# bit-bots/SoccerDiffusion

Measured on AMD Instinct MI355X. Metric: denoised joint-trajectories/s (50-step DDIM, H=100, J=20), higher is better.
Workload: dtype f32 (operands split into fp16 hi+lo, 3 fp16 MFMAs per product at every site, fp32 accumulate: 22-bit operands; single noise prediction vs the fp64 oracle 8e-7 on these weights and 2e-6 on weights stressed to |logit| ~ 60 (tests/test_gpu_denoiser.py::test_mode3_noise_prediction_single_step); valid fo; 1 GPU; BASELINE.json configs[2]: 50-step DDIM sampling, B=4096 parallel rollouts per GPU, transformer denoiser d=256 L=4 heads=4, horizon T=100, J=20, memory M=11 (10 context tokens + step token); one step = one full rollout; the timed region issues the rollout's launches eagerly.  Kernel selection: sampler mode 3 (--sampler-mode); batch_per_gpu=4096, ddim_steps=50, horizon=100, joints=20, hidden_dim=256, decoder_layers=4, parallelism=dp1 (independent rollouts, no collective)

## Files before the change

soccerdiffusion_amd/csrc/sd_traj.h:

```cpp
#pragma once
#include "sd_common.h"
#include "sd_mfma16.h"
#include "soccerdiffusion_hip.h"
#include <type_traits>

namespace tj {

constexpr int D = 256, HD = 64, NH = 4, TMAX = 100;
constexpr int NTHREADS = 512;
constexpr int MAX_L = 8;
constexpr float ACT = 8.0f;
constexpr float PSC = 1024.0f;
constexpr float XSC = 1.0f;
constexpr int XROW = 1024, X1ROW = 512, QROW = 256, VROW = 288, PROW = 512;
constexpr int LDS_X = 0;
constexpr int LDS_SQ = LDS_X + TMAX * X1ROW;
constexpr int LDS_SO = LDS_SQ + TMAX * QROW;
constexpr int LDS_Q = LDS_X + TMAX * XROW;
constexpr int LDS_K = LDS_Q + TMAX * QROW;
constexpr int LDS_P = LDS_Q;
constexpr int LDS_STAT = LDS_K + TMAX * VROW;
constexpr int LDS_BYTES = LDS_STAT + TMAX * 8 * 8;
static_assert(LDS_SO + TMAX * QROW <= LDS_Q, "Q and O fit the freed half of the panel");
static_assert(LDS_BYTES <= 163840 && LDS_P + TMAX * PROW <= LDS_STAT, "LDS budget");

typedef short s16x4 __attribute__((ext_vector_type(4)));
typedef _Float16 f16x2 __attribute__((ext_vector_type(2)));
typedef unsigned u32x4 __attribute__((ext_vector_type(4)));

#ifdef TJ_STAMPS
constexpr int TJ_NSTAMP = 96, TJ_STAMP_WGS = 512;
__device__ unsigned long long *g_tj_stamps;
#define TJ_STAMP(i)                                                                                                            \
    do {                                                                                                                       \
        if (blockIdx.x < TJ_STAMP_WGS && (threadIdx.x & 63) == 0)                                                              \
            g_tj_stamps[((long)blockIdx.x * 8 + (threadIdx.x >> 6)) * TJ_NSTAMP + (i)] = __builtin_amdgcn_s_memtime();        \
    } while (0)
template <int SITE>
__device__ __forceinline__ void tj_sync() {
    const unsigned long long t0 = __builtin_amdgcn_s_memtime();
    __syncthreads();
    const unsigned long long t1 = __builtin_amdgcn_s_memtime();
    if (blockIdx.x < TJ_STAMP_WGS && (threadIdx.x & 63) == 0) g_tj_stamps[((long)blockIdx.x * 8 + (threadIdx.x >> 6)) * TJ_NSTAMP + 64 + SITE] += t1 - t0;
}
#define TJ_SYNC(site) tj_sync<site>()
#define TJ_WAIT_FIRST_KEY() asm volatile("s_waitcnt vmcnt(28)" ::: "memory")
#else
#define TJ_STAMP(i) do {} while (0)
#define TJ_SYNC(site) __syncthreads()
#define TJ_WAIT_FIRST_KEY() do {} while (0)
#endif

#ifndef TJ_DROP_ALO
#define TJ_DROP_ALO 0
#endif
#ifndef TJ_DROP_BLO
#define TJ_DROP_BLO 0
#endif
enum Site { S_QKV = 1, S_SCORES = 2, S_PV = 4, S_OUT = 8, S_XSC = 16, S_XPV = 32, S_W1 = 64, S_W2 = 128, S_EMB = 256, S_FC = 512 };
template <int SITE = 0>
__device__ __forceinline__ void mma3(f32x4 &c, f16x8 ah, f16x8 al, f16x8 bh, f16x8 bl) {
    if constexpr ((TJ_DROP_ALO | TJ_DROP_BLO) & SITE) {
        if constexpr (!(TJ_DROP_ALO & SITE)) c = mfma16(al, bh, c);
        if constexpr (!(TJ_DROP_BLO & SITE)) c = mfma16(ah, bl, c);
        c = mfma16(ah, bh, c);
    } else {
        ::mma3(c, ah, al, bh, bl);
    }
}

__device__ __forceinline__ int kperm(int k8, int e) { return (k8 >> 2) * 32 + 16 * (e >> 2) + 4 * (k8 & 3) + (e & 3); }

static __global__ void pack_w16_kernel(const float *__restrict__ W, int N, int K, int Np, int Kp, const unsigned *maxbits, float fixed_scale,
                                f16 *__restrict__ dst, float *scale_out) {
    const float scale = maxbits ? f16_scale_from_bits(*maxbits) : fixed_scale;
    if (scale_out && blockIdx.x == 0 && threadIdx.x == 0) *scale_out = scale;
    const int nks = Kp / 32;
    const long total = (long)Np * (Kp / 8);
    for (long i = (long)blockIdx.x * blockDim.x + threadIdx.x; i < total; i += (long)gridDim.x * blockDim.x) {
        const int n = (int)(i / (Kp / 8)), k8 = (int)(i % (Kp / 8));
        f16 hh[8], ll[8];
#pragma unroll
        for (int e = 0; e < 8; ++e) {
            const int k = Kp == D ? kperm(k8, e) : k8 * 8 + e;
            const float v = (n < N && k < K) ? W[(long)n * K + k] * scale : 0.f;
            hh[e] = (f16)v;
            ll[e] = (f16)(v - (float)hh[e]);
        }
        const int nt = n >> 4, ks = k8 >> 2, lane = (k8 & 3) * 16 + (n & 15);
        f16 *o = dst + (((long)nt * nks + ks) * 2) * 512 + lane * 8;
#pragma unroll
        for (int e = 0; e < 8; ++e) {
            o[e] = hh[e];
            o[512 + e] = ll[e];
        }
    }
}

static __global__ void pack_g16_kernel(const float *__restrict__ gv, long items, int n_slots, const unsigned *maxbits, f16 *__restrict__ dst,
                                float *scale_out, int nkt = 1) {
    const float scale = f16_scale_from_bits(*maxbits);
    if (scale_out && blockIdx.x == 0 && threadIdx.x == 0) *scale_out = scale;
    const long total = items * 4 * 16 * (D / 8);
    for (long i = (long)blockIdx.x * blockDim.x + threadIdx.x; i < total; i += (long)gridDim.x * blockDim.x) {
        const int k8 = (int)(i % (D / 8)), slot = (int)((i / (D / 8)) % 16);
        const long ih = i / (D / 8) / 16;
        f16x4 h0 = {0, 0, 0, 0}, l0 = h0, h1 = h0, l1 = h0;
        if (16 * (int)((ih >> 2) % nkt) + slot < n_slots) {
            const float *row = gv + (ih * 16 + slot) * 2 * D + kperm(k8, 0);
            f16_split4(*reinterpret_cast<const f32x4 *>(row), scale, h0, l0);
            f16_split4(*reinterpret_cast<const f32x4 *>(row + 16), scale, h1, l1);
        }
        f16 *o = dst + ih * (8 * 2 * 512) + ((k8 >> 2) * 2) * 512 + ((k8 & 3) * 16 + slot) * 8;
        *reinterpret_cast<f16x4 *>(o) = h0;
        *reinterpret_cast<f16x4 *>(o + 4) = h1;
        *reinterpret_cast<f16x4 *>(o + 512) = l0;
        *reinterpret_cast<f16x4 *>(o + 516) = l1;
    }
}
static __global__ void pack_v16_kernel(const float *__restrict__ gv, long items, int n_slots, const unsigned *maxbits, f16 *__restrict__ dst,
                                float *scale_out, int nkt = 1) {
    const float scale = f16_scale_from_bits(*maxbits);
    if (scale_out && blockIdx.x == 0 && threadIdx.x == 0) *scale_out = scale;
    const long total = items * 16 * 2 * 64;
    for (long i = (long)blockIdx.x * blockDim.x + threadIdx.x; i < total; i += (long)gridDim.x * blockDim.x) {
        const int lane = (int)(i & 63), kk = (int)((i >> 6) & 1), nt = (int)((i >> 7) & 15);
        const long item = i >> 11;
        const int n = 16 * nt + (lane & 15), g = lane >> 4;
        f16 hh[8], ll[8];
#pragma unroll
        for (int e = 0; e < 8; ++e) {
            const int k = 32 * kk + 8 * g + e, head = k >> 4, slot = k & 15;
            const float v = 16 * (int)(item % nkt) + slot < n_slots ? gv[((item * 4 + head) * 16 + slot) * 2 * D + D + n] * scale : 0.f;
            hh[e] = (f16)v;
            ll[e] = (f16)(v - (float)hh[e]);
        }
        f16 *o = dst + (((item * 16 + nt) * 2 + kk) * 2) * 512 + lane * 8;
#pragma unroll
        for (int e = 0; e < 8; ++e) {
            o[e] = hh[e];
            o[512 + e] = ll[e];
        }
    }
}

struct Ctx {
    char *smem;
    int lane, w, g, t, T;
    int tok6;
    bool ok6;
    unsigned xa[4], xa6[4];
};

struct LnAffine { f32x4 w[2], b[2]; };
__device__ __forceinline__ void ln_affine_load(const Ctx &c, const float *ln_w, const float *ln_b, LnAffine &p) {
    __builtin_amdgcn_sched_barrier(0);
#pragma unroll
    for (int a = 0; a < 2; ++a) {
        p.w[a] = *reinterpret_cast<const f32x4 *>(ln_w + 32 * c.w + 16 * a + 4 * c.g);
        p.b[a] = *reinterpret_cast<const f32x4 *>(ln_b + 32 * c.w + 16 * a + 4 * c.g);
    }
    __builtin_amdgcn_sched_barrier(0);
}


template <int NSTEP, int DEPTH, class Load, class Mma>
__device__ __forceinline__ void ring_pipe(Load load, Mma mma) {
#pragma unroll
    for (int s = 0; s < DEPTH - 1; ++s)
        if (s < NSTEP) load(s);
#pragma unroll
    for (int s = 0; s < NSTEP; ++s) {
        if (s + DEPTH - 1 < NSTEP) load(s + DEPTH - 1);
        __builtin_amdgcn_sched_barrier(0);
        mma(s);
        __builtin_amdgcn_sched_barrier(0);
    }
// ... 198 lines not shown
        const f32x4 d0 = H[0][tt] - mw[tt], d1 = H[1][tt] - mw[tt];
        const f32x4 q4 = d0 * d0 + d1 * d1;
        qw[tt] = rows4_sum((q4[0] + q4[1]) + (q4[2] + q4[3]));
    }
    if (c.g == 0) {
#pragma unroll
        for (int tt = 0; tt < NTT; ++tt)
            if (tok_ok(c, tt)) *reinterpret_cast<f32x2 *>(stat + (tok_of(c, tt) * 8 + c.w) * 2) = f32x2{mw[tt], qw[tt]};
    }
    TJ_STAMP(49);
    TJ_SYNC(0);
    TJ_STAMP(50);
    char *scr = c.smem + LDS_P + c.w * 1280 + c.t * 80;
#pragma unroll
    for (int j = 0; j < (NTT > 4 ? 2 : 1); ++j) {
        const int tl = c.g + 4 * j;
        const float *sp = stat + (tl < NTT - 1 ? 16 * tl + c.t : c.tok6) * 16;
        const f32x4 p0 = *reinterpret_cast<const f32x4 *>(sp), p1 = *reinterpret_cast<const f32x4 *>(sp + 4);
        const f32x4 p2 = *reinterpret_cast<const f32x4 *>(sp + 8), p3 = *reinterpret_cast<const f32x4 *>(sp + 12);
        const float m = (((p0[0] + p0[2]) + (p1[0] + p1[2])) + ((p2[0] + p2[2]) + (p3[0] + p3[2]))) * 0.125f;
        const f32x4 e0 = f32x4{p0[0], p0[2], p1[0], p1[2]} - m, e1 = f32x4{p2[0], p2[2], p3[0], p3[2]} - m;
        const f32x4 ee = e0 * e0 + e1 * e1;
        const float m2 = (((p0[1] + p0[3]) + (p1[1] + p1[3])) + ((p2[1] + p2[3]) + (p3[1] + p3[3]))) + 32.0f * ((ee[0] + ee[1]) + (ee[2] + ee[3]));
        *reinterpret_cast<f32x2 *>(scr + 8 * tl) = f32x2{m, __builtin_amdgcn_rsqf(m2 * (1.0f / D) + SD_LN_EPS)};
    }
    __builtin_amdgcn_wave_barrier();
    float mean[NTT], rstd[NTT];
#pragma unroll
    for (int i = 0; i < (NTT + 1) / 2; ++i) {
        const f32x4 v = *reinterpret_cast<const f32x4 *>(scr + 16 * i);
        mean[2 * i] = v[0];
        rstd[2 * i] = v[1];
        if (2 * i + 1 < NTT) {
            mean[2 * i + 1] = v[2];
            rstd[2 * i + 1] = v[3];
        }
    }
    TJ_STAMP(51);
    const f32x4 gw0 = gwv[0] * ACT, gb0 = gbv[0] * ACT, gw1 = gwv[1] * ACT, gb1 = gbv[1] * ACT;
#pragma unroll
    for (int tt = 0; tt < NTT; ++tt) {
        const f32x4 y0 = ((H[0][tt] - mean[tt]) * rstd[tt]) * gw0 + gb0, y1 = ((H[1][tt] - mean[tt]) * rstd[tt]) * gw1 + gb1;
        if constexpr (HI_ONLY) store_x1(c, tt, y0, y1);
        else store_x(c, tt, y0, y1);
        if (rows_out && tok_ok(c, tt)) {
            const f32x4 u0 = y0 * (1.0f / ACT), u1 = y1 * (1.0f / ACT);
            float *at = rows_out + (long)tok_of(c, tt) * D + 32 * c.w + 4 * c.g;
            SD_NT_STORE(u0, reinterpret_cast<f32x4 *>(at));
            SD_NT_STORE(u1, reinterpret_cast<f32x4 *>(at + 16));
            if (amax) {
                const f32x4 m4 = f32x4{fmaxf(fabsf(u0[0]), fabsf(u1[0])), fmaxf(fabsf(u0[1]), fabsf(u1[1])), fmaxf(fabsf(u0[2]), fabsf(u1[2])), fmaxf(fabsf(u0[3]), fabsf(u1[3]))};
                *amax = fmaxf(*amax, fmaxf(fmaxf(m4[0], m4[1]), fmaxf(m4[2], m4[3])));
            }
        }
        __builtin_amdgcn_sched_barrier(0);
    }
    TJ_STAMP(52);
    TJ_SYNC(1);
}
template <bool HI_ONLY = false>
static __device__ __forceinline__ void layer_norm_to_x(const Ctx &c0, const f32x4 (&H)[2][NTT], const float *ln_w, const float *ln_b, float *rows_out = nullptr,
                                                       float *amax = nullptr) {
    LnAffine aff;
    ln_affine_load(c0, ln_w, ln_b, aff);
    layer_norm_to_x<HI_ONLY>(c0, H, aff, rows_out, amax);
}

template <int T0 = 0, int NT = NTT, class Body>
static __device__ __forceinline__ void gemm_pipe(const Ctx &c, const f16 *pa0, const f16 *pa1, Body body) {
    const char *X = c.smem + LDS_X;
    const unsigned lo = (unsigned)c.lane * 8;
    f16x8 a0[2][2], a1[2][2], b[2][2];
#pragma unroll
    for (int pl = 0; pl < 2; ++pl) {
        a0[0][pl] = *reinterpret_cast<const f16x8 *>(pa0 + lo + pl * 512);
        a1[0][pl] = *reinterpret_cast<const f16x8 *>(pa1 + lo + pl * 512);
        b[0][pl] = lds16(X + x_at(c, T0, pl, 0));
    }
#pragma unroll
    for (int ks = 0; ks < 8; ++ks) {
#pragma unroll
        for (int tt = T0; tt < T0 + NT; ++tt) {
            const int cur = (ks * NT + tt - T0) & 1, nxt = cur ^ 1;
            if (tt == T0 && ks + 1 < 8) {
#pragma unroll
                for (int pl = 0; pl < 2; ++pl) {
                    a0[(ks + 1) & 1][pl] = *reinterpret_cast<const f16x8 *>(pa0 + lo + ((ks + 1) * 2 + pl) * 512);
                    a1[(ks + 1) & 1][pl] = *reinterpret_cast<const f16x8 *>(pa1 + lo + ((ks + 1) * 2 + pl) * 512);
                }
            }
            const int nks = tt + 1 < T0 + NT ? ks : ks + 1, ntt = tt + 1 < T0 + NT ? tt + 1 : T0;
            if (nks < 8) {
#pragma unroll
                for (int pl = 0; pl < 2; ++pl) b[nxt][pl] = lds16(X + x_at(c, ntt, pl, nks));
            }
            __builtin_amdgcn_sched_barrier(0);
            body(tt, a0[ks & 1][0], a0[ks & 1][1], a1[ks & 1][0], a1[ks & 1][1], b[cur][0], b[cur][1]);
            __builtin_amdgcn_sched_barrier(0);
        }
    }
}

struct HeadAcc { f32x4 a0[NTT], a1[NH0]; };
template <bool odd>
static __device__ __forceinline__ void gemm_head(const Ctx &c, HeadAcc &acc, const f16 *pa0, const f16 *pa1) {
    const char *X = c.smem + LDS_X;
    const unsigned lo = (unsigned)c.lane * 8;
    f16x8 a0[2][2], a1[2][2], b[2];
#pragma unroll
    for (int pl = 0; pl < 2; ++pl) {
        a0[0][pl] = *reinterpret_cast<const f16x8 *>(pa0 + lo + pl * 512);
        a1[0][pl] = *reinterpret_cast<const f16x8 *>(pa1 + lo + pl * 512);
    }
    b[0] = lds16(X + x1_at(c, 0, 0));
#pragma unroll
    for (int ks = 0; ks < 8; ++ks) {
#pragma unroll
        for (int tt = 0; tt < NTT; ++tt) {
            const int cur = (ks * NTT + tt) & 1, nxt = cur ^ 1;
            if (tt == 0 && ks + 1 < 8) {
#pragma unroll
                for (int pl = 0; pl < 2; ++pl) {
                    a0[(ks + 1) & 1][pl] = *reinterpret_cast<const f16x8 *>(pa0 + lo + ((ks + 1) * 2 + pl) * 512);
                    a1[(ks + 1) & 1][pl] = *reinterpret_cast<const f16x8 *>(pa1 + lo + ((ks + 1) * 2 + pl) * 512);
                }
            }
            const int nks = tt + 1 < NTT ? ks : ks + 1, ntt = tt + 1 < NTT ? tt + 1 : 0;
            if (nks < 8) b[nxt] = lds16(X + x1_at(c, ntt, nks));
            __builtin_amdgcn_sched_barrier(0);
            acc.a0[tt] = mfma16(a0[ks & 1][1], b[cur], acc.a0[tt]);
            acc.a0[tt] = mfma16(a0[ks & 1][0], b[cur], acc.a0[tt]);
            if constexpr (!odd) {
                if (tt < NH0) {
                    acc.a1[tt] = mfma16(a1[ks & 1][1], b[cur], acc.a1[tt]);
                    acc.a1[tt] = mfma16(a1[ks & 1][0], b[cur], acc.a1[tt]);
                }
            } else if (tt >= NH0) {
                acc.a1[tt - NH0] = mfma16(a1[ks & 1][1], b[cur], acc.a1[tt - NH0]);
                acc.a1[tt - NH0] = mfma16(a1[ks & 1][0], b[cur], acc.a1[tt - NH0]);
            }
            __builtin_amdgcn_sched_barrier(0);
        }
    }
}

template <int SITE>
static __device__ __forceinline__ void gemm_x2(const Ctx &c, f32x4 (&acc)[2][NTT], const f16 *wmat) {
    const f16 *pa = wmat + (long)(2 * c.w) * (8 * 2 * 512);
    gemm_pipe(c, pa, pa + 8 * 2 * 512, [&](int tt, f16x8 a0h, f16x8 a0l, f16x8 a1h, f16x8 a1l, f16x8 bh, f16x8 bl) __attribute__((always_inline)) {
        mma3<SITE>(acc[0][tt], a0h, a0l, bh, bl);
        mma3<SITE>(acc[1][tt], a1h, a1l, bh, bl);
    });
}

static __device__ __forceinline__ void gemm_k64(const Ctx &c, f32x4 (&acc)[2][NTT], const AK64 &f, const char *Bbuf) {
    const f16x8 (&a)[2][2][2] = f.a;
    f16x8 b[3][2];
    ring_pipe<2 * NTT, 3>(
        [&](int s) __attribute__((always_inline)) {
            b[s % 3][0] = lds16(Bbuf + q_at(c, s >> 1, 0, s & 1));
            b[s % 3][1] = lds16(Bbuf + q_at(c, s >> 1, 1, s & 1));
        },
        [&](int s) __attribute__((always_inline)) {
            const int tt = s >> 1, kk = s & 1;
            mma3<S_OUT>(acc[0][tt], a[0][kk][0], a[0][kk][1], b[s % 3][0], b[s % 3][1]);
            mma3<S_OUT>(acc[1][tt], a[1][kk][0], a[1][kk][1], b[s % 3][0], b[s % 3][1]);
        });
}


static __device__ __forceinline__ void head_zero(HeadAcc &acc) {
#pragma unroll
    for (int tt = 0; tt < NTT; ++tt) acc.a0[tt] = f32x4{0.f, 0.f, 0.f, 0.f};
#pragma unroll
    for (int i = 0; i < NH0; ++i) acc.a1[i] = f32x4{0.f, 0.f, 0.f, 0.f};
}
static __device__ __forceinline__ void head_gemm(const Ctx &c0, const SaW &a, int h, HeadAcc &acc) {
    const Ctx c = ctx_local(c0);
    const int w = c.w;
    const int nt0 = (w < 4 ? 0 : 16) + 4 * h + (w & 3);
    const int nt1 = 32 + 4 * h + (w >> 1);
    head_zero(acc);
    if (w & 1) gemm_head<true>(c, acc, a.w_in + (long)nt0 * (8 * 2 * 512), a.w_in + (long)nt1 * (8 * 2 * 512));
    else gemm_head<false>(c, acc, a.w_in + (long)nt0 * (8 * 2 * 512), a.w_in + (long)nt1 * (8 * 2 * 512));
}
static __device__ __forceinline__ void head_write_qkv(const Ctx &c0, const SaW &a, int h, const HeadAcc &acc) {
    const Ctx c = ctx_local(c0);
    const int w = c.w, g = c.g, t = c.t, w3 = w & 3;
    const float c_in = 1.0f / a.s_in;
    {
        const f32x4 bv = *reinterpret_cast<const f32x4 *>(a.b_in + (w < 4 ? 0 : D) + HD * h + 16 * w3 + 4 * g) * ACT;
        char *dst = c.smem + (w < 4 ? LDS_SQ : LDS_Q);
        const int chunk = (2 * (w3 & 1) + (g >> 1)) | ((w3 >> 1) << 3);
#pragma unroll
        for (int tt = 0; tt < NTT; ++tt) {
            if (!tok_ok(c, tt)) continue;
            const int tok = tok_of(c, tt);
            split_store(dst + q_off(tok, chunk) + 8 * (g & 1), dst + q_off(tok, chunk | 4) + 8 * (g & 1), acc.a0[tt] * c_in + bv);
            __builtin_amdgcn_sched_barrier(0);
        }
    }
    {
        const f32x4 bv = *reinterpret_cast<const f32x4 *>(a.b_in + 2 * D + HD * h + 16 * (w >> 1) + 4 * g) * ACT;
        const int tt1 = (w & 1) ? NH0 : 0, n1 = (w & 1) ? NTT - NH0 : NH0;
#pragma unroll
        for (int i = 0; i < NH0; ++i) {
            if (i >= n1) continue;
            const int tok = 16 * (tt1 + i) + t;
            if (tok >= c.T) continue;
            char *at = c.smem + LDS_K + tok * VROW + 2 * (16 * (w >> 1) + 4 * g);
            split_store(at, at + 128, acc.a1[i] * c_in + bv);
        }
    }
}
static __device__ __forceinline__ void att_scores(const Ctx &c, const SaW &a, const char *Qb, const char *Kb, f32x4 (&S)[NTT], float &psum,
                                                  float *lse2 = nullptr) {
    const int w = c.w, g = c.g, t = c.t;
    {
        f16x8 qf[2][2];
        const int qtok = min(16 * w + t, c.T - 1);
#pragma unroll
        for (int kk = 0; kk < 2; ++kk)
#pragma unroll
            for (int pl = 0; pl < 2; ++pl) qf[kk][pl] = lds16(Qb + q_off(qtok, g | (pl << 2) | (kk << 3)));
#pragma unroll
        for (int kt = 0; kt < NTT; ++kt) S[kt] = f32x4{0.f, 0.f, 0.f, 0.f};
        f16x8 kf[4][2];
        ring_pipe<2 * NTT, 4>(
            [&](int s) __attribute__((always_inline)) {
                kf[s & 3][0] = lds16(Kb + q_at(c, s >> 1, 0, s & 1));
                kf[s & 3][1] = lds16(Kb + q_at(c, s >> 1, 1, s & 1));
            },
            [&](int s) __attribute__((always_inline)) { mma3<S_SCORES>(S[s >> 1], kf[s & 3][0], kf[s & 3][1], qf[s & 1][0], qf[s & 1][1]); });
    }
    const float c_s = a.scale_log2e / (ACT * ACT);
#pragma unroll
    for (int r = 0; r < 4; ++r)
        if (LAST0 + 4 * g + r >= c.T) S[NTT - 1][r] = -INFINITY;
    f32x4 m4 = S[0];
#pragma unroll
    for (int kt = 1; kt < NTT; ++kt) m4 = f32x4{fmaxf(m4[0], S[kt][0]), fmaxf(m4[1], S[kt][1]), fmaxf(m4[2], S[kt][2]), fmaxf(m4[3], S[kt][3])};
    const float m = rows4_max(fmaxf(fmaxf(m4[0], m4[1]), fmaxf(m4[2], m4[3])));
    if constexpr (!PRECISE) {
        if (a.status && __builtin_amdgcn_ballot_w64(fabsf(m) * c_s > SD_SHARP_LOGIT_LIMIT * 1.44269504088896340736f) != 0) {
            if (c.lane == 0) atomicOr(a.status, SD_STATUS_SHARP_LOGITS);
        }
    }
    const float mb = m * c_s - 10.0f;
    f32x4 ps = {0.f, 0.f, 0.f, 0.f};
#pragma unroll
    for (int kt = 0; kt < NTT; ++kt) {
        const f32x4 e = S[kt] * c_s - mb;
        S[kt] = f32x4{__builtin_amdgcn_exp2f(e[0]), __builtin_amdgcn_exp2f(e[1]), __builtin_amdgcn_exp2f(e[2]), __builtin_amdgcn_exp2f(e[3])};
        ps = ps + S[kt];
    }
    psum = rows4_sum((ps[0] + ps[1]) + (ps[2] + ps[3]));
    if (lse2) *lse2 = mb + __builtin_amdgcn_logf(psum);
}
template <bool SPLIT_UNDER = false>
static __device__ __forceinline__ void att_pv(const Ctx &c, const f32x4 (&S)[NTT], float psum, const char *Vb, char *Ob, float *rows_out = nullptr,
                                              int ld = 0, float *amax = nullptr) {
    const int w = c.w, g = c.g, t = c.t;
    f32x4 O[4];
#pragma unroll
    for (int ft = 0; ft < 4; ++ft) O[ft] = f32x4{0.f, 0.f, 0.f, 0.f};
    const int q4 = t >> 2, p4 = t & 3;
    const auto vload = [&](int s, f16x8 (&vf)[4][2]) __attribute__((always_inline)) {
        const int kp = s >> 2, ft = s & 3;
        const int r0 = min(32 * kp + 4 * g + q4, c.T - 1), r1 = min(32 * kp + 16 + 4 * g + q4, c.T - 1);
        const char *v0 = Vb + r0 * VROW + 8 * p4, *v1 = Vb + r1 * VROW + 8 * p4;
#pragma unroll
        for (int pn = 0; pn < 2; ++pn) {
            const s16x4 x0 = __builtin_amdgcn_ds_read_tr16_b64_v4i16((__attribute__((address_space(3))) s16x4 *)(v0 + pn * 128 + ft * 32));
            const s16x4 x1 = __builtin_amdgcn_ds_read_tr16_b64_v4i16((__attribute__((address_space(3))) s16x4 *)(v1 + pn * 128 + ft * 32));
            vf[s & 3][pn] = __builtin_shufflevector(__builtin_bit_cast(f16x4, x0), __builtin_bit_cast(f16x4, x1), 0, 1, 2, 3, 4, 5, 6, 7);
        }
    };
    if constexpr (SPLIT_UNDER) {
        f16x8 vf[4][2];
        unsigned ph[2][4], pl[2][4];
        const auto psplit = [&](int kp, int q) __attribute__((always_inline)) {
            const int kt = 2 * kp + (q >> 1);
            f16x2 h = {0, 0}, l = {0, 0};
            if (kt < NTT) {
                const f32x2 x = {S[kt < NTT ? kt : 0][2 * (q & 1)], S[kt < NTT ? kt : 0][2 * (q & 1) + 1]};
                h = __builtin_convertvector(x, f16x2);
                l = __builtin_convertvector(x - __builtin_convertvector(h, f32x2), f16x2);
            }
            ph[kp & 1][q] = __builtin_bit_cast(unsigned, h);
            pl[kp & 1][q] = __builtin_bit_cast(unsigned, l);
            if (kt < NTT) asm volatile("" : "+v"(ph[kp & 1][q]), "+v"(pl[kp & 1][q]));
        };
        const auto pfrag = [](const unsigned (&p)[4]) __attribute__((always_inline)) { return __builtin_bit_cast(f16x8, u32x4{p[0], p[1], p[2], p[3]}); };
#pragma unroll
        for (int q = 0; q < 4; ++q) psplit(0, q);
#pragma unroll
        for (int s = 0; s < 3; ++s) vload(s, vf);
#pragma unroll
        for (int s = 0; s < 4 * NKP; ++s) {
            const int kp = s >> 2;
            if (s + 3 < 4 * NKP) vload(s + 3, vf);
            __builtin_amdgcn_sched_barrier(0);
            mma3<S_PV>(O[s & 3], vf[s & 3][0], vf[s & 3][1], pfrag(ph[kp & 1]), pfrag(pl[kp & 1]));
            if (kp + 1 < NKP) {
                psplit(kp + 1, s & 3);
#pragma unroll
// ... 288 lines not shown
#pragma unroll
        for (int i = 0; i < NH0; ++i) {
            if (i >= n1) continue;
            const f32x4 p = S[kt][i];
            const int tt = tt1 + i, tok = tt < NTT - 1 ? 16 * tt + c.t : c.tok6;
            if (tt == NTT - 1 && !c.ok6) continue;
            const int chunk = (2 * (hh & 1) + (c.g >> 1)) | ((hh >> 1) << 3);
            split_store(Pb + p_off(tok, chunk) + 8 * (c.g & 1), Pb + p_off(tok, chunk | 4) + 8 * (c.g & 1), p * ss.m_c);
            if (kt == klast && c.g == (mcs >> 2)) {
                const float pv = p[mcs & 3] * ss.m_s;
                const f16 ph = (f16)pv, pl = (f16)(pv - (float)ph);
                const f16x8 z8h = {ph, 0, 0, 0, 0, 0, 0, 0}, z8l = {pl, 0, 0, 0, 0, 0, 0, 0};
                *reinterpret_cast<f16x8 *>(Pb + p_off(tok, hh | (2 << 3))) = z8h;
                *reinterpret_cast<f16x8 *>(Pb + p_off(tok, hh | 4 | (2 << 3))) = z8l;
            }
        }
        f16x8 av[2][3][2];
#pragma unroll
        for (int n = 0; n < 2; ++n) {
            const f16 *vp = L.v16 + (((traj * nkt + kt) * 16 + 2 * c.w + n) * 2) * (2 * 512) + c.lane * 8;
#pragma unroll
            for (int kk = 0; kk < 2; ++kk)
#pragma unroll
                for (int pl = 0; pl < 2; ++pl) av[n][kk][pl] = *reinterpret_cast<const f16x8 *>(vp + (kk * 2 + pl) * 512);
#pragma unroll
            for (int pl = 0; pl < 2; ++pl) {
                const f16 sv = vstep[(pl * 4 + c.g) * D + 16 * (2 * c.w + n) + c.t];
                av[n][2][pl] = f16x8{sv, 0, 0, 0, 0, 0, 0, 0};
            }
        }
        TJ_SYNC(5);
        f16x8 pb[3][2];
        if (kt == klast) {
            ring_pipe<3 * NTT, 3>(
                [&](int s) __attribute__((always_inline)) {
                    pb[s % 3][0] = lds16(Pb + p_at(c, s / 3, 0, s % 3));
                    pb[s % 3][1] = lds16(Pb + p_at(c, s / 3, 1, s % 3));
                },
                [&](int s) __attribute__((always_inline)) {
                    const int tt = s / 3, kk = s % 3;
                    mma3<S_XPV>(H[0][tt], av[0][kk][0], av[0][kk][1], pb[s % 3][0], pb[s % 3][1]);
                    mma3<S_XPV>(H[1][tt], av[1][kk][0], av[1][kk][1], pb[s % 3][0], pb[s % 3][1]);
                });
        } else {
            ring_pipe<2 * NTT, 3>(
                [&](int s) __attribute__((always_inline)) {
                    pb[s % 3][0] = lds16(Pb + p_at(c, s / 2, 0, s % 2));
                    pb[s % 3][1] = lds16(Pb + p_at(c, s / 2, 1, s % 2));
                },
                [&](int s) __attribute__((always_inline)) {
                    const int tt = s / 2, kk = s % 2;
                    mma3<S_XPV>(H[0][tt], av[0][kk][0], av[0][kk][1], pb[s % 3][0], pb[s % 3][1]);
                    mma3<S_XPV>(H[1][tt], av[1][kk][0], av[1][kk][1], pb[s % 3][0], pb[s % 3][1]);
                });
        }
    }
    unscale_h(H, 1.0f / up, boc);
}

template <bool WIDE = false>
static __device__ __forceinline__ void decoder_layer(const Ctx &c0, const LayerW &L, f32x4 (&H)[2][NTT], long traj, int Mk, float scale_log2e, int *status,
                                                     int nkt = 1, long sblk = 0) {
    const f16 *gstep = L.gstep + sblk * STEP_G_HALFS, *vstep = L.vstep + sblk * STEP_V_HALFS;
    {
        const Ctx &c = c0;
        const float s_o = L.sc[0], up = ACT * s_o;
        scale_h(H, up);
        Bias2 bo;
        const SaW sw{L.w_in, L.b_in, L.w_o, L.sc[3], scale_log2e, status};
        if constexpr (PRECISE) sa_block_precise(c, sw, H, L.b_o, bo);
        else sa_block(c, sw, H, L.b_o, bo);
        unscale_h(H, 1.0f / up, bo);
    }
    TJ_STAMP(31);
    LnAffine aff2;
    ln_affine_load(c0, L.n2_w, L.n2_b, aff2);
    float sc4 = 0.f, sc5 = 0.f, sc6 = 0.f, sc7 = 0.f;
    if constexpr (!WIDE) {
        sc4 = L.sc[4], sc5 = L.sc[5], sc6 = L.sc[6], sc7 = L.sc[7];
    }
    f16x8 gfr[8][2];
    if constexpr (!WIDE) {
        const int hh = c0.w >> 1, Mc = Mk - 1;
        const f16 *gp = c0.t == Mc ? gstep + (long)hh * (8 * 2 * 32) + c0.g * 8 : L.g16 + (traj * 4 + hh) * (8 * 2 * 512) + c0.lane * 8;
        const int gstride = c0.t == Mc ? 32 : 512;
        __builtin_amdgcn_sched_barrier(0);
#pragma unroll
        for (int ks = 0; ks < 8; ++ks)
#pragma unroll
            for (int pl = 0; pl < 2; ++pl) gfr[ks][pl] = *reinterpret_cast<const f16x8 *>(gp + (ks * 2 + pl) * gstride);
        __builtin_amdgcn_sched_barrier(0);
    }
    layer_norm_to_x(c0, H, aff2);
    TJ_STAMP(32);
    if constexpr (WIDE) {
        cross_wide(c0, L, H, traj, Mk, nkt, scale_log2e, sblk);
    } else {
        const Ctx c = ctx_local(c0);
        const int hh = c.w >> 1, Mc = Mk - 1;
        const bool odd = c.w & 1;
        const int tt1 = odd ? NH0 : 0, n1 = odd ? NTT - NH0 : NH0;
        char *Pb = c.smem + LDS_P;
        const char *X = c.smem + LDS_X;
        f32x4 S[NH0];
#pragma unroll
        for (int i = 0; i < NH0; ++i) S[i] = f32x4{0.f, 0.f, 0.f, 0.f};
        const auto uni = [](float v) __attribute__((always_inline)) { return __builtin_bit_cast(float, __builtin_amdgcn_readfirstlane(__builtin_bit_cast(int, v))); };
        sc4 = uni(sc4), sc5 = uni(sc5), sc6 = uni(sc6), sc7 = uni(sc7);
        f32x4 cbv = *reinterpret_cast<const f32x4 *>(L.cb + traj * 64 + hh * 16 + 4 * c.g);
        const float cs = L.cstep[sblk * 4 + hh];
        __builtin_amdgcn_sched_barrier(0);
        f16x8 av[2][3][2];
        f16 svv[2][2];
#pragma unroll
        for (int n = 0; n < 2; ++n) {
            const f16 *vp = L.v16 + ((traj * 16 + 2 * c.w + n) * 2) * (2 * 512) + c.lane * 8;
#pragma unroll
            for (int kk = 0; kk < 2; ++kk)
#pragma unroll
                for (int pl = 0; pl < 2; ++pl) av[n][kk][pl] = *reinterpret_cast<const f16x8 *>(vp + (kk * 2 + pl) * 512);
#pragma unroll
            for (int pl = 0; pl < 2; ++pl) svv[n][pl] = vstep[(pl * 4 + c.g) * D + 16 * (2 * c.w + n) + c.t];
        }
        __builtin_amdgcn_sched_barrier(0);
        auto scores = [&](auto odd_c) __attribute__((always_inline)) {
            constexpr bool OD = decltype(odd_c)::value;
            constexpr int N1 = OD ? NTT - NH0 : NH0, T1 = OD ? NH0 : 0;
            constexpr int N1D = N1 > 0 ? N1 : 1;
            f16x8 xb[3][2];
            ring_pipe<8 * N1, 3>(
                [&](int s) __attribute__((always_inline)) {
                    xb[s % 3][0] = lds16(X + x_at(c, T1 + s % N1D, 0, s / N1D));
                    xb[s % 3][1] = lds16(X + x_at(c, T1 + s % N1D, 1, s / N1D));
                },
                [&](int s) __attribute__((always_inline)) { mma3<S_XSC>(S[s % N1D], gfr[s / N1D][0], gfr[s / N1D][1], xb[s % 3][0], xb[s % 3][1]); });
        };
        TJ_WAIT_FIRST_KEY();
        TJ_STAMP(53);
        if (odd) scores(std::true_type{});
        else scores(std::false_type{});
#pragma unroll
        for (int n = 0; n < 2; ++n)
#pragma unroll
            for (int pl = 0; pl < 2; ++pl) av[n][2][pl] = f16x8{svv[n][pl], 0, 0, 0, 0, 0, 0, 0};
        const float c_g = 1.0f / (ACT * sc4);
        const StepScale ss = step_scale(sc5, sc6, sc7);
        f32x4 cg4 = {c_g, c_g, c_g, c_g};
#pragma unroll
        for (int r = 0; r < 4; ++r)
            if (4 * c.g + r == Mc) {
                cbv[r] = cs;
                cg4[r] = ss.c_gs;
            }
        TJ_SYNC(4);
#pragma unroll
        for (int i = 0; i < NH0; ++i) {
            if (i >= n1) continue;
            f32x4 v = S[i] * cg4 + cbv;
#pragma unroll
            for (int r = 0; r < 4; ++r)
                if (4 * c.g + r >= Mk) v[r] = -INFINITY;
            const float m = rows4_max(fmaxf(fmaxf(v[0], v[1]), fmaxf(v[2], v[3])));
            const f32x4 e = (v - m) * scale_log2e;
            f32x4 p = {__builtin_amdgcn_exp2f(e[0]), __builtin_amdgcn_exp2f(e[1]), __builtin_amdgcn_exp2f(e[2]), __builtin_amdgcn_exp2f(e[3])};
            const float sum = rows4_sum((p[0] + p[1]) + (p[2] + p[3]));
            const float f = PSC / sum;
            const float pstep = p[Mc & 3] * (f * ss.m_s);
            p = p * (f * ss.m_c);
            const int tt = tt1 + i, tok = tt < NTT - 1 ? 16 * tt + c.t : c.tok6;
            if (tt == NTT - 1 && !c.ok6) continue;
            const int chunk = (2 * (hh & 1) + (c.g >> 1)) | ((hh >> 1) << 3);
            split_store(Pb + p_off(tok, chunk) + 8 * (c.g & 1), Pb + p_off(tok, chunk | 4) + 8 * (c.g & 1), p);
            if (c.g == (Mc >> 2)) {
                const float pv = pstep;
                const f16 ph = (f16)pv, pl = (f16)(pv - (float)ph);
                const f16x8 z8h = {ph, 0, 0, 0, 0, 0, 0, 0}, z8l = {pl, 0, 0, 0, 0, 0, 0, 0};
                *reinterpret_cast<f16x8 *>(Pb + p_off(tok, hh | (2 << 3))) = z8h;
                *reinterpret_cast<f16x8 *>(Pb + p_off(tok, hh | 4 | (2 << 3))) = z8l;
            }
        }
        TJ_SYNC(5);
        TJ_STAMP(33);
        const float up = PSC * ss.s_v;
        const Bias2 boc = bias_load(c, L.b_oc);
        scale_h(H, up);
        f16x8 pb[3][2];
        ring_pipe<3 * NTT, 3>(
            [&](int s) __attribute__((always_inline)) {
                pb[s % 3][0] = lds16(Pb + p_at(c, s / 3, 0, s % 3));
                pb[s % 3][1] = lds16(Pb + p_at(c, s / 3, 1, s % 3));
            },
            [&](int s) __attribute__((always_inline)) {
                const int tt = s / 3, kk = s % 3;
                mma3<S_XPV>(H[0][tt], av[0][kk][0], av[0][kk][1], pb[s % 3][0], pb[s % 3][1]);
                mma3<S_XPV>(H[1][tt], av[1][kk][0], av[1][kk][1], pb[s % 3][0], pb[s % 3][1]);
            });
        unscale_h(H, 1.0f / up, boc);
    }
    TJ_STAMP(34);
    layer_norm_to_x(c0, H, L.n3_w, L.n3_b);
    TJ_STAMP(35);
    {
        const Ctx c = ctx_local(c0);
        f32x4 U[2][NTT];
#pragma unroll
        for (int a = 0; a < 2; ++a)
#pragma unroll
            for (int tt = 0; tt < NTT; ++tt) U[a][tt] = f32x4{0.f, 0.f, 0.f, 0.f};
        const float sc1 = L.sc[1];
        const Bias2 b1 = bias_load(c, L.b_1);
        gemm_x2<S_W1>(c, U, L.w_1);
        TJ_STAMP(36);
        const float c1 = 1.0f / (ACT * sc1);
        const float sc2 = L.sc[2];
        const Bias2 b2 = bias_load(c, L.b_2);
        TJ_SYNC(6);
#pragma unroll
        for (int tt = 0; tt < NTT; ++tt) {
            f32x4 gl[2];
#pragma unroll
            for (int a = 0; a < 2; ++a) {
                const f32x4 pre = U[a][tt] * c1 + b1.v[a];
                const f32x2 g0 = gelu_erf_as2(f32x2{pre[0], pre[1]}) * ACT, g1 = gelu_erf_as2(f32x2{pre[2], pre[3]}) * ACT;
                gl[a] = f32x4{g0[0], g0[1], g1[0], g1[1]};
            }
            store_x(c, tt, gl[0], gl[1]);
            __builtin_amdgcn_sched_barrier(0);
        }
        TJ_SYNC(7);
        TJ_STAMP(37);
        const float up = ACT * sc2;
        scale_h(H, up);
        gemm_x2<S_W2>(c, H, L.w_2);
        unscale_h(H, 1.0f / up, b2);
    }
    TJ_STAMP(38);
    if (L.nln_w) layer_norm_to_x<!PRECISE>(c0, H, L.nln_w, L.nln_b);
    TJ_STAMP(39);
}

static __device__ __forceinline__ float ddim_update(float x, float e, const f32x4 &k) {
    const float x0 = __builtin_fmaf(-k[1], e, x) / k[0];
    const float ce = k[3] * e;
    return __builtin_fmaf(k[2], x0, ce);
}

template <bool WIDE = false, int PIN = 0, bool ROLL = false, bool DRAWS = false>
static __device__ __forceinline__ void step_body(const StepArgs &a, const PinArgs &pin = PinArgs{}, f32x4 roll_coef = f32x4{0.f, 0.f, 0.f, 0.f},
                                                 int roll_step = 0, int roll_wave = 0, int draws = 1, const HoldArgs &hold = HoldArgs{},
                                                 const MultistepArgs &ms = MultistepArgs{}, const LimitArgs &lim = LimitArgs{},
                                                 const SlewArgs &sl = SlewArgs{}, const DirectArgs &dr = DirectArgs{}) {
    constexpr bool HOLD = PIN == 2;
    constexpr bool MS = PIN == 3;
    constexpr bool LIM = PIN == 4;
    constexpr bool ACCEL = PIN == 7;
    constexpr bool SLEW = PIN == 5 || ACCEL;
    constexpr bool DIRECT = PIN == 6;
    static_assert(!(SLEW || DIRECT) || TMAX * 128 + TMAX * 4 <= LDS_STAT - LDS_Q, "the slew twin's S and M planes fit the Q | K region");
    extern __shared__ __attribute__((aligned(16))) char smem[];
    Ctx c;
    if constexpr (ROLL) c = ctx_fresh(smem, roll_wave, a.T);
    else ctx_init(c, smem, a.T);
    const long traj = blockIdx.x;
    const long cidx = DRAWS ? (long)((unsigned)blockIdx.x / (unsigned)draws) : traj;
    const int J = a.J;
    TJ_STAMP(0);
    f32x4 H[2][NTT];
    {
        char *Qb = c.smem + LDS_Q;
        f16x8 we[2][2];
        f32x4 be[2], pe4[2][NTT];
#pragma unroll
        for (int n = 0; n < 2; ++n) {
            const f16 *wp = a.w_emb + (long)(2 * c.w + n) * (2 * 512) + c.lane * 8;
            we[n][0] = *reinterpret_cast<const f16x8 *>(wp);
            we[n][1] = *reinterpret_cast<const f16x8 *>(wp + 512);
            const int n0 = 32 * c.w + 16 * n + 4 * c.g;
            be[n] = *reinterpret_cast<const f32x4 *>(a.b_emb + n0);
#pragma unroll
            for (int tt = 0; tt < NTT; ++tt) pe4[n][tt] = *reinterpret_cast<const f32x4 *>(a.pe + (long)tok_of(c, tt) * D + n0);
        }
        __builtin_amdgcn_sched_barrier(0);
        const float *xr = a.x + traj * (long)a.T * J;
        const int tid = ROLL ? 64 * c.w + c.lane : (int)threadIdx.x;
        if constexpr (ACCEL) {
            float *xs = reinterpret_cast<float *>(c.smem + LDS_X);
            for (int tok = tid; tok < a.T; tok += NTHREADS) xs[TMAX + tok] = x_token_scale(xr + tok * J, J, xs + tok);
            __syncthreads();
        }
        if (J & 3) {
            for (int i = tid; i < a.T * 4; i += NTHREADS) {
                const int tok = i >> 2, chunk = i & 3;
                f16x8 h8, l8;
                if constexpr (ACCEL) {
                    const float xs = reinterpret_cast<const float *>(c.smem + LDS_X)[TMAX + tok];
#pragma unroll
                    for (int e = 0; e < 8; ++e) {
                        const int j = 8 * chunk + e;
                        const float v = j < J ? xr[tok * J + j] * XSC * xs : 0.f;
                        h8[e] = (f16)v;
                        l8[e] = (f16)(v - (float)h8[e]);
                    }
                    *reinterpret_cast<f16x8 *>(Qb + q_off(tok, chunk)) = h8;
                    *reinterpret_cast<f16x8 *>(Qb + q_off(tok, chunk | 4)) = l8;
                    continue;
                }
#pragma unroll
                for (int e = 0; e < 8; ++e) {
                    const int j = 8 * chunk + e;
                    const float v = j < J ? xr[tok * J + j] * XSC : 0.f;
                    h8[e] = (f16)v;
                    l8[e] = (f16)(v - (float)h8[e]);
                }
                *reinterpret_cast<f16x8 *>(Qb + q_off(tok, chunk)) = h8;
                *reinterpret_cast<f16x8 *>(Qb + q_off(tok, chunk | 4)) = l8;
            }
        }
        const int nvec = (J & 3) ? 0 : a.T * J / 4;
        for (int i = tid; i < nvec; i += NTHREADS) {
            const f32x4 v = *reinterpret_cast<const f32x4 *>(xr + 4 * i) * XSC;
            const int tok = (4 * i) / J, j0 = 4 * i - tok * J;
            const int chunk = j0 >> 3;
            if constexpr (ACCEL) {
                const float xs = reinterpret_cast<const float *>(c.smem + LDS_X)[TMAX + tok];
                split_store(Qb + q_off(tok, chunk) + 2 * (j0 & 7), Qb + q_off(tok, chunk | 4) + 2 * (j0 & 7), v * xs);
            } else {
                split_store(Qb + q_off(tok, chunk) + 2 * (j0 & 7), Qb + q_off(tok, chunk | 4) + 2 * (j0 & 7), v);
            }
            if (j0 + 4 >= J) {
                const f16x4 z4 = {0, 0, 0, 0};
                for (int k = J; k < 32; k += 4) {
                    *reinterpret_cast<f16x4 *>(Qb + q_off(tok, k >> 3) + 2 * (k & 7)) = z4;
                    *reinterpret_cast<f16x4 *>(Qb + q_off(tok, (k >> 3) | 4) + 2 * (k & 7)) = z4;
                }
            }
        }
        TJ_SYNC(8);
        const float c_e = 1.0f / (XSC * a.sc_io[0]);
#pragma unroll
        for (int n = 0; n < 2; ++n) {
            const f16x8 ah = we[n][0], al = we[n][1];
#pragma unroll
            for (int tt = 0; tt < NTT; ++tt) {
                f32x4 acc = {0.f, 0.f, 0.f, 0.f};
                mma3<S_EMB>(acc, ah, al, lds16(Qb + q_at(c, tt, 0, 0)), lds16(Qb + q_at(c, tt, 1, 0)));
                if constexpr (ACCEL) {
                    H[n][tt] = acc * (c_e * reinterpret_cast<const float *>(c.smem + LDS_X)[tok_of(c, tt)]) + (be[n] + pe4[n][tt]);
                    continue;
                }
                H[n][tt] = acc * c_e + (be[n] + pe4[n][tt]);
            }
        }
    }
    TJ_STAMP(1);
    layer_norm_to_x<!PRECISE>(c, H, a.n1_w, a.n1_b);
    TJ_STAMP(2);
#pragma unroll 1
    for (int l = 0; l < a.L; ++l) decoder_layer<WIDE>(c, a.layer[l], H, cidx, a.Mk, a.scale_log2e, a.status, a.nkt,
                                                           ROLL ? (long)roll_step : a.step_per_traj ? (a.step_map ? (long)a.step_map[traj] : traj) : 0L);
    const Ctx &c_step = c;
    {
        Ctx c_tail;
        if constexpr (ROLL) c_tail = ctx_fresh(smem, roll_wave, a.T);
        const Ctx &c = ROLL ? c_tail : c_step;
        float *stat = reinterpret_cast<float *>(c.smem + LDS_STAT);
        int pin_rows = 0;
        if constexpr (PIN == 1) pin_rows = (!DRAWS || pin.rows) ? pin.rows[traj] : 0;
        float am[NTT];
#pragma unroll
        for (int tt = 0; tt < NTT; ++tt) {
            const f32x4 a0 = H[0][tt], a1 = H[1][tt];
            float m = fmaxf(fmaxf(fabsf(a0[0]), fabsf(a0[1])), fmaxf(fabsf(a0[2]), fabsf(a0[3])));
            m = fmaxf(m, fmaxf(fmaxf(fabsf(a1[0]), fabsf(a1[1])), fmaxf(fabsf(a1[2]), fabsf(a1[3]))));
            am[tt] = rows4_max(m);
        }
        if (c.g == 0) {
#pragma unroll
            for (int tt = 0; tt < NTT; ++tt)
                if (tok_ok(c, tt)) stat[tok_of(c, tt) * 8 + c.w] = am[tt];
        }
        TJ_SYNC(9);
#pragma unroll
        for (int tt = 0; tt < NTT; ++tt) {
            const float *sp = stat + tok_of(c, tt) * 8;
            const f32x4 p0 = *reinterpret_cast<const f32x4 *>(sp), p1 = *reinterpret_cast<const f32x4 *>(sp + 4);
            const float m = fmaxf(fmaxf(fmaxf(p0[0], p0[1]), fmaxf(p0[2], p0[3])), fmaxf(fmaxf(p1[0], p1[1]), fmaxf(p1[2], p1[3])));
            const float s = f16_scale_from_bits(__builtin_bit_cast(unsigned, m));
// ... 575 lines not shown
```

Measured before the change: 16020 trajectories/s.

## Split FFN W2 GEMM into two k-halves staged across separate LDS buffers

Result: no change. 16090 trajectories/s (median of 6 runs) (+0.5%).

```diff
diff --git a/soccerdiffusion_amd/csrc/sd_traj.h b/soccerdiffusion_amd/csrc/sd_traj.h
--- a/soccerdiffusion_amd/csrc/sd_traj.h
+++ b/soccerdiffusion_amd/csrc/sd_traj.h
@@ -23,6 +23,13 @@
 constexpr int LDS_BYTES = LDS_STAT + TMAX * 8 * 8;
 static_assert(LDS_SO + TMAX * QROW <= LDS_Q, "Q and O fit the freed half of the panel");
 static_assert(LDS_BYTES <= 163840 && LDS_P + TMAX * PROW <= LDS_STAT, "LDS budget");
+
+#ifndef TJ_FFN_SPLIT
+#define TJ_FFN_SPLIT 1
+#endif
+#ifndef TJ_XATTN_SYNC_P
+#define TJ_XATTN_SYNC_P 0
+#endif
 
 typedef short s16x4 __attribute__((ext_vector_type(4)));
 typedef _Float16 f16x2 __attribute__((ext_vector_type(2)));
@@ -527,6 +534,47 @@
         mma3<SITE>(acc[1][tt], a1h, a1l, bh, bl);
     });
 }
+
+#if TJ_FFN_SPLIT
+template <int SITE, int KS0>
+static __device__ __forceinline__ void gemm_x2_half(const Ctx &c, f32x4 (&acc)[2][NTT], const f16 *wmat) {
+    static_assert(KS0 == 0 || KS0 == 4, "a k half");
+    const f16 *pa0 = wmat + (long)(2 * c.w) * (8 * 2 * 512), *pa1 = pa0 + 8 * 2 * 512;
+    const char *Bb = c.smem + (KS0 == 0 ? LDS_P : LDS_X);
+    const auto b_at = [&](int tt, int pl, int ks) __attribute__((always_inline)) { return KS0 == 0 ? p_at(c, tt, pl, ks) : x_at(c, tt, pl, ks); };
+    const unsigned lo = (unsigned)c.lane * 8;
+    f16x8 a0[2][2], a1[2][2], b[2][2];
+#pragma unroll
+    for (int pl = 0; pl < 2; ++pl) {
+        a0[0][pl] = *reinterpret_cast<const f16x8 *>(pa0 + lo + (KS0 * 2 + pl) * 512);
+        a1[0][pl] = *reinterpret_cast<const f16x8 *>(pa1 + lo + (KS0 * 2 + pl) * 512);
+        b[0][pl] = lds16(Bb + b_at(0, pl, KS0));
+    }
+#pragma unroll
+    for (int ks = KS0; ks < KS0 + 4; ++ks) {
+#pragma unroll
+        for (int tt = 0; tt < NTT; ++tt) {
+            const int cur = ((ks - KS0) * NTT + tt) & 1, nxt = cur ^ 1;
+            if (tt == 0 && ks + 1 < KS0 + 4) {
+#pragma unroll
+                for (int pl = 0; pl < 2; ++pl) {
+                    a0[(ks + 1) & 1][pl] = *reinterpret_cast<const f16x8 *>(pa0 + lo + ((ks + 1) * 2 + pl) * 512);
+                    a1[(ks + 1) & 1][pl] = *reinterpret_cast<const f16x8 *>(pa1 + lo + ((ks + 1) * 2 + pl) * 512);
+                }
+            }
+            const int nks = tt + 1 < NTT ? ks : ks + 1, ntt = tt + 1 < NTT ? tt + 1 : 0;
+            if (nks < KS0 + 4) {
+#pragma unroll
+                for (int pl = 0; pl < 2; ++pl) b[nxt][pl] = lds16(Bb + b_at(ntt, pl, nks));
+            }
+            __builtin_amdgcn_sched_barrier(0);
+            mma3<SITE>(acc[0][tt], a0[ks & 1][0], a0[ks & 1][1], b[cur][0], b[cur][1]);
+            mma3<SITE>(acc[1][tt], a1[ks & 1][0], a1[ks & 1][1], b[cur][0], b[cur][1]);
+            __builtin_amdgcn_sched_barrier(0);
+        }
+    }
+}
+#endif
 
 static __device__ __forceinline__ void gemm_k64(const Ctx &c, f32x4 (&acc)[2][NTT], const AK64 &f, const char *Bbuf) {
     const f16x8 (&a)[2][2][2] = f.a;
@@ -1121,7 +1169,9 @@
                 cbv[r] = cs;
                 cg4[r] = ss.c_gs;
             }
+#if TJ_XATTN_SYNC_P
         TJ_SYNC(4);
+#endif
 #pragma unroll
         for (int i = 0; i < NH0; ++i) {
             if (i >= n1) continue;
@@ -1183,6 +1233,50 @@
         const float c1 = 1.0f / (ACT * sc1);
         const float sc2 = L.sc[2];
         const Bias2 b2 = bias_load(c, L.b_2);
+#if TJ_FFN_SPLIT
+        const float up = ACT * sc2;
+        const bool lowq = c.w < 4;
+        const unsigned gbase = lowq ? (unsigned)LDS_P : (unsigned)LDS_X;
+        const int gshift = lowq ? 9 : 10;
+        static_assert(PROW == 1 << 9 && XROW == 1 << 10, "row pitches as shifts");
+        if (!lowq) {
+            TJ_SYNC(6);
+            TJ_STAMP(55);
+        }
+#pragma unroll
+        for (int tt = 0; tt < NTT; ++tt) {
+            f32x4 gl[2];
+#pragma unroll
+            for (int a = 0; a < 2; ++a) {
+                const f32x4 pre = U[a][tt] * c1 + b1.v[a];
+                const f32x2 g0 = gelu_erf_as2(f32x2{pre[0], pre[1]}) * ACT, g1 = gelu_erf_as2(f32x2{pre[2], pre[3]}) * ACT;
+                gl[a] = f32x4{g0[0], g0[1], g1[0], g1[1]};
+            }
+            if (tok_ok(c, tt)) {
+                const int chunk = c.g | (c.w << 3), tok = tok_of(c, tt);
+                char *row = c.smem + gbase + ((unsigned)tok << gshift);
+                split_store8(row + ((chunk ^ (tok & 15)) << 4), row + (((chunk | 4) ^ (tok & 15)) << 4), gl[0], gl[1]);
+            }
+            __builtin_amdgcn_sched_barrier(0);
+        }
+        TJ_STAMP(54);
+        if (lowq) {
+            TJ_SYNC(6);
+            TJ_STAMP(55);
+        } else {
+            TJ_SYNC(7);
+            TJ_STAMP(37);
+        }
+        scale_h(H, up);
+        gemm_x2_half<S_W2, 0>(c, H, L.w_2);
+        TJ_STAMP(58);
+        if (lowq) {
+            TJ_SYNC(7);
+            TJ_STAMP(37);
+        }
+        gemm_x2_half<S_W2, 4>(c, H, L.w_2);
+        unscale_h(H, 1.0f / up, b2);
+#else
         TJ_SYNC(6);
 #pragma unroll
         for (int tt = 0; tt < NTT; ++tt) {
@@ -1202,6 +1296,7 @@
         scale_h(H, up);
         gemm_x2<S_W2>(c, H, L.w_2);
         unscale_h(H, 1.0f / up, b2);
+#endif
     }
     TJ_STAMP(38);
     if (L.nln_w) layer_norm_to_x<!PRECISE>(c0, H, L.nln_w, L.nln_b);
```
